# gk969/stm32-speech-recognition

Measured on NVIDIA H100. Metric: utterances/s, higher is better.
Workload: dtype int32 fixed-point (s16 FFT, u32 energies)

## Files before the change

stm32-speech-recognition_b200/csrc/sr_mfcc.cu:

```cuda
#include <stdio.h>
#include "sr_mfcc_core.cuh"

namespace srk {

constexpr int kPcmBufBytes = 19264;
__host__ __device__ constexpr int padF(int e) { return e + ((e >> 6) << 2); }
constexpr int kFftWords = 2 * (padF(1023) + 1);
static_assert(kFftWords >= kFftWordsTotal, "filter scratch must fit in the FFT buffer");

constexpr int kMfccWarps = 16;
constexpr int kNBuf = 3;

struct __align__(16) MfccSmem {
    unsigned char pcm[kNBuf][kPcmBufBytes];
    int2 tw[340 * 3];
    u32 log_thr[2220];
    u32 tri_even[512];
    u32 tri_odd[512];
    int4 dct[24 * 3];
    u32 fftbuf[kMfccWarps][kFftWords];
    s32 wq[kMfccWarps][160];
    u32 lg[kMfccWarps][32];
    u64 full[kNBuf];
    u64 empty[kNBuf];
    s32 meta[kNBuf][5];
    int turn;
};

static_assert(sizeof(MfccSmem) <= 232448, "mfcc_kernel_s16 exceeds the 227 KB shared-memory opt-in limit");

__device__ __forceinline__ void stage_utterance(MfccSmem &sm, int it, u32 b, const u16 *__restrict__ pcm,
                                                u32 U, const u32 *__restrict__ seg, u32 seg_stride,
                                                const atap_tag *__restrict__ atap, unsigned char *__restrict__ ftr,
                                                const u32 *__restrict__ row_map, size_t total_bytes, bool base_aligned,
                                                int lane) {
    const int s = it % kNBuf;
    const u32 st = seg[(size_t)b * seg_stride], en = seg[(size_t)b * seg_stride + 1];
    const u32 mid = atap[b].mid_val;
    const long long row = row_map ? (long long)row_map[b] : (long long)b;
    if (it >= kNBuf) mbar_wait(&sm.empty[s], ((it / kNBuf) - 1) & 1);
    const int F = mfcc_frames<SR_FRAME_LEN>(st, en, U);
    if (lane == 0) *reinterpret_cast<u16 *>(ftr + (size_t)b * kFtrBytes + 2) = (u16)F;
    if (F == 0) {
        if (lane == 0) {
            sm.meta[s][0] = 0; sm.meta[s][1] = 0; sm.meta[s][2] = (s32)mid; sm.meta[s][3] = (s32)b; sm.meta[s][4] = 0;
            mbar_arrive(&sm.full[s]);
        }
        return;
    }
    if (lane == 0) sm.meta[s][4] = (st == 0);
    long long first = row * U + st - 1;
    const long long last = row * U + st + 80ll * (F - 1) + 160;
    unsigned char *dst = sm.pcm[s];
    int off = 0;
    if (first < 0) {
        first = 0; off = 8;
        dst += 16;
    }
    const size_t lo = (size_t)first * 2, hi = (size_t)last * 2;
    if (base_aligned) {
        const size_t lo_al = lo & ~(size_t)15;
        size_t hi_al = (hi + 15) & ~(size_t)15;
        const size_t lim = total_bytes & ~(size_t)15;
        if (hi_al > lim) hi_al = lim;
        const u32 nbytes = (u32)(hi_al - lo_al);
        const int shift = (int)((lo - lo_al) >> 1);
        if (lane == 0) {
            sm.meta[s][0] = F; sm.meta[s][2] = (s32)mid; sm.meta[s][3] = (s32)b;
            sm.meta[s][1] = (off ? 7 : shift);
        }
        if (hi > hi_al) {
            const u16 *g = reinterpret_cast<const u16 *>(reinterpret_cast<const unsigned char *>(pcm) + hi_al);
            u16 *d = reinterpret_cast<u16 *>(dst + (hi_al - lo_al));
            const int n = (int)((hi - hi_al) >> 1);
            if (lane < n) d[lane] = g[lane];
        }
        __syncwarp();
        if (lane == 0) {
            mbar_arrive_expect_tx(&sm.full[s], nbytes);
            bulk_g2s(dst, reinterpret_cast<const unsigned char *>(pcm) + lo_al, nbytes, &sm.full[s]);
        }
    } else {
        const u16 *g = pcm + first;
        u16 *d = reinterpret_cast<u16 *>(dst);
        const int n = (int)(last - first);
        for (int i = lane; i < n; i += 32) d[i] = g[i];
        __syncwarp();
        if (lane == 0) {
            sm.meta[s][0] = F; sm.meta[s][2] = (s32)mid; sm.meta[s][1] = off ? 7 : 0; sm.meta[s][3] = (s32)b;
            mbar_arrive(&sm.full[s]);
        }
    }
}

__device__ __forceinline__ void stage_end(MfccSmem &sm, int it, int lane) {
    const int s = it % kNBuf;
    if (it >= kNBuf) mbar_wait(&sm.empty[s], ((it / kNBuf) - 1) & 1);
    if (lane == 0) { sm.meta[s][0] = -1; mbar_arrive(&sm.full[s]); }
}

__global__ void __maxnreg__(128) mfcc_kernel_s16(const u16 *__restrict__ pcm, u32 U, u32 B, const u32 *__restrict__ seg,
                                                 u32 seg_stride, const atap_tag *__restrict__ atap,
                                                 unsigned char *__restrict__ ftr, const DevTables *__restrict__ tab,
                                                 const u32 *__restrict__ row_map, u32 rows_total, const u32 *__restrict__ B_dev,
                                                 u32 *__restrict__ work ) {
    constexpr int kAhead = kNBuf - 2;
    if (B_dev) B = min(B, *B_dev);
    auto cta_done = [&]() {
        if (work && threadIdx.x == 0) {
            __threadfence();
            if (atomicAdd(&work[1], 1u) == gridDim.x - 1u) { work[0] = 0; work[1] = 0; }
        }
    };
    if (blockIdx.x >= B) { cta_done(); return; }
    extern __shared__ __align__(128) unsigned char smem_raw[];
    MfccSmem &sm = *reinterpret_cast<MfccSmem *>(smem_raw);
    const int warp = threadIdx.x >> 5, lane = threadIdx.x & 31;

    for (int i = threadIdx.x; i < 340 * 3; i += blockDim.x) sm.tw[i] = tab->tw[i];
    for (int i = threadIdx.x; i < 2220; i += blockDim.x) sm.log_thr[i] = tab->log_thr[i];
    for (int i = threadIdx.x; i < 24 * 12; i += blockDim.x)
        reinterpret_cast<s32 *>(sm.dct)[i] = (s32)tab->dct[(i / 24) * 24 + ((i / 12) & 1) * 12 + i % 12];
    for (int i = threadIdx.x; i < 512; i += blockDim.x) {
        sm.tri_even[flt_word(i >> 4, i & 15)] = tab->tri_even[i];
        sm.tri_odd[flt_word(i >> 4, i & 15)] = tab->tri_odd[i];
    }
    if (threadIdx.x == 0) {
        for (int s = 0; s < kNBuf; ++s) { mbar_init(&sm.full[s], 1); mbar_init(&sm.empty[s], kMfccWarps); }
        sm.turn = 0;
        mbar_fence_init();
    }
    __syncthreads();

    const size_t total_bytes = (size_t)(row_map ? rows_total : B) * U * 2;
    const bool base_aligned = (reinterpret_cast<uintptr_t>(pcm) & 15) == 0;

    auto claim_stage = [&](int it_s) {
        u32 b;
        if (work) {
            b = 0;
            if (lane == 0) {
                volatile int *turn = &sm.turn;
                while (*turn != it_s) { }
                b = atomicAdd(&work[0], 1u);
                __threadfence_block();
                if (b != 0xFFFFFFFFu) *turn = it_s + 1;
            }
            b = __shfl_sync(0xFFFFFFFFu, b, 0);
        }
        else b = blockIdx.x + (u32)it_s * gridDim.x;
        if (b < B) stage_utterance(sm, it_s, b, pcm, U, seg, seg_stride, atap, ftr, row_map, total_bytes, base_aligned, lane);
        else stage_end(sm, it_s, lane);
    };
    if (warp < kAhead) claim_stage(warp);

    u32 *fb = sm.fftbuf[warp];
    s32 *wq = sm.wq[warp];
    const int q1 = lane & 3;
    const int2 k1_2 = sm.tw[q1 * 3 + 1], k1_1 = sm.tw[q1 * 3 + 2];
    int2 k2t[4][3];
#pragma unroll
    for (int m1 = 0; m1 < 4; ++m1)
#pragma unroll
        for (int j = 0; j < 3; ++j) k2t[m1][j] = sm.tw[(4 + q1 + 4 * m1) * 3 + j];
    const u32 hm0 = tab->hamm[lane], hm1 = tab->hamm[lane + 32], hm2 = tab->hamm[lane + 64],
              hm3 = tab->hamm[lane + 96], hm4 = tab->hamm[lane + 128];
    const int fsw = (lane >> 1) & 3;
    int fe_lo = kFltZero, fe_hi = kFltZero, fx_lo = kFltX, fx_hi = kFltX;
    if (lane < 24) {
        fe_lo = tab->flt_e_lo[lane]; fe_hi = tab->flt_e_hi[lane];
        fx_lo = kFltX + (lane & 1) * 33 + tab->flt_x_lo[lane]; fx_hi = kFltX + (lane & 1) * 33 + tab->flt_x_hi[lane];
    }
    const int4 *dctk4 = sm.dct + 3 * (lane < 24 ? lane : 0);

    u32 gidx = 0;
    for (int it = 0;; ++it) {
        if (warp == it % kMfccWarps) claim_stage(it + kAhead);
        const int s = it % kNBuf;
        mbar_wait(&sm.full[s], (it / kNBuf) & 1);
        const int F = sm.meta[s][0];
        if (F < 0) break;
        const u32 b = (u32)sm.meta[s][3];
        const int off = sm.meta[s][1];
        const s32 mid = sm.meta[s][2];
        u16 *x = reinterpret_cast<u16 *>(sm.pcm[s]) + off;
        unsigned char *out_rows = ftr + (size_t)b * kFtrBytes + 4;
        const int f0 = (int)((warp - (int)(gidx % kMfccWarps) + kMfccWarps) % kMfccWarps);
        if (f0 == 0 && lane == 0 && sm.meta[s][4]) x[0] = (u16)mid;

        auto preemph = [&](const u16 *xf) {
            const u32 hm[5] = {hm0, hm1, hm2, hm3, hm4};
#pragma unroll
            for (int k = 0; k < 5; ++k) {
                const int i = lane + 32 * k;
                wq[i] = preemph_hamm(xf[i + 1], xf[i], (u32)mid, hm[k]) >> 2;
            }
        };
        for (int f = f0; f < F; f += kMfccWarps) {
            const u16 *xf = x + 80 * f;
            preemph(xf);
            __syncwarp();

#pragma unroll 1
            for (int pass = 0; pass < 2; ++pass) {
                const int G = (lane >> 2) + 8 * pass;
                const int r0 = (int)(__brev((u32)G) >> 28);
                u32 vr[4][4], vi[4][4];
#pragma unroll
                for (int m2 = 0; m2 < 4; ++m2) {
                    const int r = r0 + 16 * (((m2 & 1) << 1) | (m2 >> 1));
                    const u32 a = (u32)wq[r];
                    const u32 c = (u32)wq[r + 64];
                    u32 Cr, Ci, Br = 0, Bi = 0;
                    cxmul(Cr, Ci, c, 0u, (u32)k1_2.x, (u32)k1_2.y);
                    if ((m2 & 1) == 0) {
                        const u32 bb = (u32)wq[r + 128];
                        cxmul(Br, Bi, bb, 0u, (u32)k1_1.x, (u32)k1_1.y);
                    }
                    u32 o[8];
                    cxadda4<14>(a, 0u, Br, Bi, Cr, Ci, 0u, 0u, o[0], o[1], o[2], o[3], o[4], o[5], o[6], o[7]);
#pragma unroll
                    for (int m1 = 0; m1 < 4; ++m1) { vr[m2][m1] = o[2 * m1]; vi[m2][m1] = o[2 * m1 + 1]; }
                }
#pragma unroll
                for (int m1 = 0; m1 < 4; ++m1) {
                    const int q2 = q1 + 4 * m1;
                    const int2 k3 = k2t[m1][0], k2 = k2t[m1][1], k1 = k2t[m1][2];
                    u32 Dr, Di, Cr, Ci, Br, Bi;
                    cxmul(Dr, Di, vr[3][m1], vi[3][m1], (u32)k3.x, (u32)k3.y);
                    cxmul(Cr, Ci, vr[2][m1], vi[2][m1], (u32)k2.x, (u32)k2.y);
                    cxmul(Br, Bi, vr[1][m1], vi[1][m1], (u32)k1.x, (u32)k1.y);
                    u32 o[8];
                    cxadda4<14>(vr[0][m1], vi[0][m1], Br, Bi, Cr, Ci, Dr, Di, o[0], o[1], o[2], o[3], o[4], o[5], o[6], o[7]);
                    uint2 *dst = reinterpret_cast<uint2 *>(fb) + padF(64 * G + q2);
#pragma unroll
                    for (int m = 0; m < 4; ++m) dst[16 * m] = make_uint2(o[2 * m], o[2 * m + 1]);
                }
            }
            __syncwarp();

            u32 held[8];
#pragma unroll
            for (int pass = 0; pass < 2; ++pass) {
                const int q3 = lane + 32 * pass;
                u32 vr[4][4], vi[4][4];
                const int2 *k = &sm.tw[(20 + q3) * 3];
                const int2 k3 = k[0], k2 = k[1], k1 = k[2];
                const uint2 *pts = reinterpret_cast<const uint2 *>(fb) + padF(q3);
#pragma unroll
                for (int m4 = 0; m4 < 4; ++m4) {
                    u32 pr[4], pi[4];
#pragma unroll
                    for (int m3 = 0; m3 < 4; ++m3) {
                        const uint2 p = pts[padF(256 * m4 + 64 * m3)];
                        pr[m3] = p.x; pi[m3] = p.y;
                    }
                    u32 Dr, Di, Cr, Ci, Br, Bi;
                    cxmul(Dr, Di, pr[3], pi[3], (u32)k3.x, (u32)k3.y);
                    cxmul(Cr, Ci, pr[2], pi[2], (u32)k2.x, (u32)k2.y);
                    cxmul(Br, Bi, pr[1], pi[1], (u32)k1.x, (u32)k1.y);
                    u32 o[8];
                    cxadda4<14>(pr[0], pi[0], Br, Bi, Cr, Ci, Dr, Di, o[0], o[1], o[2], o[3], o[4], o[5], o[6], o[7]);
#pragma unroll
                    for (int m3 = 0; m3 < 4; ++m3) { vr[m4][m3] = o[2 * m3]; vi[m4][m3] = o[2 * m3 + 1]; }
                }
                __syncwarp();
                if (pass == 1) {
#pragma unroll
                    for (int m3 = 0; m3 < 4; ++m3) { fb[padF(lane + 64 * m3)] = held[2 * m3]; fb[padF(lane + 64 * m3 + 256)] = held[2 * m3 + 1]; }
                }
#pragma unroll
                for (int m3 = 0; m3 < 4; ++m3) {
                    const int q4 = q3 + 64 * m3;
                    const int2 *kk = &sm.tw[(84 + q4) * 3];
                    const int2 j3 = kk[0], j2 = kk[1], j1 = kk[2];
                    u32 Dr, Di, Cr, Ci, Br, Bi;
                    cxmul(Dr, Di, vr[3][m3], vi[3][m3], (u32)j3.x, (u32)j3.y);
                    cxmul(Cr, Ci, vr[2][m3], vi[2][m3], (u32)j2.x, (u32)j2.y);
                    cxmul(Br, Bi, vr[1][m3], vi[1][m3], (u32)j1.x, (u32)j1.y);
                    u32 o[8];
                    cxadda4<14>(vr[0][m3], vi[0][m3], Br, Bi, Cr, Ci, Dr, Di, o[0], o[1], o[2], o[3], o[4], o[5], o[6], o[7]);
                    const u32 m0 = mag10_small(o[0], o[1]);
                    const u32 m1 = mag10_small(o[2], o[3]);
                    if (pass == 0) { held[2 * m3] = m0 * m0; held[2 * m3 + 1] = m1 * m1; }
                    else { fb[padF(q4)] = m0 * m0; fb[padF(q4 + 256)] = m1 * m1; }
                }
            }
            __syncwarp();

            {
                u32 E[16];
                const uint4 *e4 = reinterpret_cast<const uint4 *>(fb + 16 * lane + 4 * (lane >> 2));
#pragma unroll
                for (int j = 0; j < 4; ++j) { const uint4 v = e4[j]; E[4 * j] = v.x; E[4 * j + 1] = v.y; E[4 * j + 2] = v.z; E[4 * j + 3] = v.w; }
                __syncwarp();
                const uint4 *we4 = reinterpret_cast<const uint4 *>(sm.tri_even + 16 * lane);
                const uint4 *wo4 = reinterpret_cast<const uint4 *>(sm.tri_odd + 16 * lane);
                uint4 *re4 = reinterpret_cast<uint4 *>(fb + 16 * lane);
                uint4 *ro4 = reinterpret_cast<uint4 *>(fb + kFltRowWords + 16 * lane);
                u32 te = 0, to = 0;
#pragma unroll
                for (int j = 0; j < 4; ++j) {
                    const uint4 we = we4[j ^ fsw], wo = wo4[j ^ fsw];
                    uint4 pe, po;
                    pe.x = te; te += (E[4 * j] * we.x) / 100u;      po.x = to; to += (E[4 * j] * wo.x) / 100u;
                    pe.y = te; te += (E[4 * j + 1] * we.y) / 100u;  po.y = to; to += (E[4 * j + 1] * wo.y) / 100u;
                    pe.z = te; te += (E[4 * j + 2] * we.z) / 100u;  po.z = to; to += (E[4 * j + 2] * wo.z) / 100u;
                    pe.w = te; te += (E[4 * j + 3] * we.w) / 100u;  po.w = to; to += (E[4 * j + 3] * wo.w) / 100u;
                    re4[j ^ fsw] = pe; ro4[j ^ fsw] = po;
                }
                fb[kFltX + lane] = te;
                fb[kFltX + 33 + lane] = to;
                fb[kFltZero] = 0u;
            }
            __syncwarp();
            {
                u32 acc = fb[fe_hi] - fb[fe_lo];
#pragma unroll
                for (int j = 0; j < 6; ++j) if (fx_lo + j < fx_hi) acc += fb[fx_lo + j];
                sm.lg[warp][lane] = (lane < 24) ? log100(acc, sm.log_thr) : 0u;
            }
            __syncwarp();
            {
                const int4 d0 = dctk4[0], d1 = dctk4[1], d2 = dctk4[2];
                const s32 dctk[12] = {d0.x, d0.y, d0.z, d0.w, d1.x, d1.y, d1.z, d1.w, d2.x, d2.y, d2.z, d2.w};
                dct_row(sm.lg[warp], dctk, out_rows + (size_t)f * kRowBytes, lane);
            }
            __syncwarp();
        }
        gidx += (u32)F;
        __syncwarp();
        if (lane == 0) mbar_arrive(&sm.empty[s]);
    }
    __syncthreads();
    cta_done();
}

__global__ void __launch_bounds__(128)
fft_generic_kernel(const u32 *__restrict__ in , const s16 *__restrict__ frames, u32 len,
                   u32 n, u32 *__restrict__ raw_out , u32 *__restrict__ mag ,
                   const DevTables *__restrict__ tab) {
    __shared__ u32 buf[4][1024];
    __shared__ u32 src[4][1024];
    const int warp = threadIdx.x >> 5, lane = threadIdx.x & 31;
    const u32 fr = blockIdx.x * 4 + warp;
    if (fr >= n) return;
    u32 *x = src[warp], *y = buf[warp];
    for (int i = lane; i < 1024; i += 32) {
        u32 v;
        if (in) v = in[(size_t)fr * 1024 + i];
        else v = (u32)i < len ? (u32)(u16)frames[(size_t)fr * len + i] : 0u;
        x[i] = v;
    }
    __syncwarp();
    fft_radix4<1024>(x, y, tab, lane);
    if (raw_out) for (int i = lane; i < 1024; i += 32) raw_out[(size_t)fr * 1024 + i] = y[i];
    if (mag) for (int i = lane; i < 512; i += 32) mag[(size_t)fr * 512 + i] = mag10(lo16s(y[i]), hi16s(y[i]));
}

cudaError_t launch_mfcc(const u16 *pcm, u32 U, u32 B, const u32 *seg, u32 seg_stride, const atap_tag *atap,
                        void *ftr, int num_sms, cudaStream_t st, const u32 *row_map, u32 rows_total, const u32 *B_dev, u32 *work) {
    if (B == 0) return cudaSuccess;
    const DevTables *tab = dev_tables();
    if (!tab) return cudaErrorInitializationError;
    const size_t smem = sizeof(MfccSmem);
    const int threads = kMfccWarps * 32;
    cudaError_t e = cudaFuncSetAttribute(mfcc_kernel_s16, cudaFuncAttributeMaxDynamicSharedMemorySize, (int)smem);
    if (e != cudaSuccess) return e;
    const u32 grid = B < (u32)num_sms ? B : (u32)num_sms;
    mfcc_kernel_s16<<<grid, threads, smem, st>>>(pcm, U, B, seg, seg_stride, atap, static_cast<unsigned char *>(ftr), tab,
                                                 row_map, rows_total, B_dev, work);
    e = cudaGetLastError();
    if (e != cudaSuccess) {
        cudaFuncAttributes fa;
        if (cudaFuncGetAttributes(&fa, mfcc_kernel_s16) == cudaSuccess)
            fprintf(stderr, "mfcc kernel launch failed (%s): regs %d, maxThreads %d, static smem %zu, dyn smem %zu (max %d), threads %d\n",
                    cudaGetErrorString(e), fa.numRegs, fa.maxThreadsPerBlock, fa.sharedSizeBytes, smem,
                    fa.maxDynamicSharedSizeBytes, threads);
    }
    return e;
}

cudaError_t launch_fft_generic(const u32 *in_packed, const s16 *frames, u32 len, u32 n, u32 *raw_out, u32 *mag,
                               cudaStream_t st) {
    if (n == 0) return cudaSuccess;
    const DevTables *tab = dev_tables();
    if (!tab) return cudaErrorInitializationError;
    fft_generic_kernel<<<(n + 3) / 4, 128, 0, st>>>(in_packed, frames, len, n, raw_out, mag, tab);
    return cudaGetLastError();
}

}
```

stm32-speech-recognition_b200/csrc/sr_mfcc_core.cuh:

```cuda
#pragma once
#include "sr_common.cuh"

namespace srk {

template <u32 kFrameLen>
__device__ __forceinline__ int mfcc_frames(u32 start, u32 end, u32 U) {
    if (start == SR_SEG_NULL || end == SR_SEG_NULL || end > U || start > end) return 0;
    u32 len = end - start;
    if (len < kFrameLen) return 0;
    u32 n = (len - kFrameLen) / SR_FRAME_MOV + 1u;
    return n > SR_VV_FRM_MAX ? 0 : (int)n;
}

__device__ __forceinline__ s32 preemph_hamm(u32 cur, u32 prv, u32 mid, u32 hamm) {
    const s32 c = (s32)(cur - mid), p = (s32)(prv - mid);
    const s32 t = (s32)((u32)c - (u32)((s32)((u32)p * 95u) / 100));
    return (s32)(s16)((s32)((u32)t * hamm) / 1000);
}

template <int N>
__device__ __forceinline__ void fft_radix4(const u32 *x, u32 *y, const DevTables *tab, int lane) {
    static_assert(N == 256 || N == 1024, "the twiddle table serves N = 256 and 1024");
    constexpr int kQ = N / 4, kRevShift = N == 256 ? 26 : 24;
    for (int idx = lane; idx < kQ; idx += 32) {
        const int j = (int)(__brev((u32)idx) >> kRevShift);
        const u32 A = x[j], C = x[j + kQ], Bv = x[j + 2 * kQ], D = x[j + 3 * kQ];
        u32 o[8];
        cxadda4<0>(lo16s(A), hi16s(A), lo16s(Bv), hi16s(Bv), lo16s(C), hi16s(C), lo16s(D), hi16s(D),
                   o[0], o[1], o[2], o[3], o[4], o[5], o[6], o[7]);
#pragma unroll
        for (int m = 0; m < 4; ++m) y[4 * idx + m] = pack16(o[2 * m], o[2 * m + 1]);
    }
    __syncwarp();
    int toff = 0;
    for (int s = 4; s <= kQ; s <<= 2) {
        for (int t = lane; t < kQ; t += 32) {
            const int q = t % s, base = (t / s) * 4 * s;
            const int2 k3 = tab->tw[(toff + q) * 3], k2 = tab->tw[(toff + q) * 3 + 1], k1 = tab->tw[(toff + q) * 3 + 2];
            const u32 p0 = y[base + q], p1 = y[base + q + s], p2 = y[base + q + 2 * s], p3 = y[base + q + 3 * s];
            u32 Dr, Di, Cr, Ci, Br, Bi, o[8];
            cxmul(Dr, Di, lo16s(p3), hi16s(p3), (u32)k3.x, (u32)k3.y);
            cxmul(Cr, Ci, lo16s(p2), hi16s(p2), (u32)k2.x, (u32)k2.y);
            cxmul(Br, Bi, lo16s(p1), hi16s(p1), (u32)k1.x, (u32)k1.y);
            cxadda4<14>(lo16s(p0), hi16s(p0), Br, Bi, Cr, Ci, Dr, Di, o[0], o[1], o[2], o[3], o[4], o[5], o[6], o[7]);
#pragma unroll
            for (int m = 0; m < 4; ++m) y[base + q + m * s] = pack16(o[2 * m], o[2 * m + 1]);
        }
        __syncwarp();
        toff += s;
    }
}

__device__ __forceinline__ u32 log100(u32 v, const u32 *thr) {
    if (v == 0) return 0;
    int L = (int)(__log2f(__uint2float_rn(v)) * 69.31471805599453f);
    L = max(0, min(L, 2218));
    while (v < thr[L]) --L;
    while (L < 2218 && v >= thr[L + 1]) ++L;
    return (u32)L;
}

__device__ __forceinline__ void dct_row(const u32 *lg, const s32 (&w)[12], unsigned char *row, int lane) {
    const u32 *lgp = lg + (lane & 1) * 12;
    s32 acc = 0;
#pragma unroll
    for (int i = 0; i < 12; ++i) acc += ((s32)lgp[i] * w[i]) / 100;
    acc += __shfl_xor_sync(0xFFFFFFFFu, acc, 1);
    if (lane < 24 && (lane & 1) == 0) *reinterpret_cast<s16 *>(row + (lane >> 1) * 2) = (s16)acc;
}

}
```

Before: 11.39 million.

## Batch log and DCT tail across frames with mulhi-based division

Filterbank energies are buffered per warp for four frames, then log100 and the DCT run as one batch so all 32 lanes do useful work instead of 24. The per-term divide by 100 in the DCT becomes a __mulhi with pre-scaled weights plus a count of negative terms as a rounding correction. log100 gets branchless single-step corrections, and the window buffer shrinks to s16 with explicit sign-extending loads. The single-step correction assumes the float estimate is off by at most one, and the mulhi trick must reproduce truncating division exactly.

Result: faster. 11.56 million (median of 6 runs) (+1.5%).

```diff
diff --git a/stm32-speech-recognition_b200/csrc/sr_mfcc.cu b/stm32-speech-recognition_b200/csrc/sr_mfcc.cu
--- a/stm32-speech-recognition_b200/csrc/sr_mfcc.cu
+++ b/stm32-speech-recognition_b200/csrc/sr_mfcc.cu
@@ -5,11 +5,17 @@
 
 constexpr int kPcmBufBytes = 19264;
 __host__ __device__ constexpr int padF(int e) { return e + ((e >> 6) << 2); }
+__device__ __forceinline__ u32 lds_s16(const s16 *p) {
+    s32 v;
+    asm volatile("ld.shared.s16 %0, [%1];" : "=r"(v) : "r"(smem_u32(p)) : "memory");
+    return (u32)v;
+}
 constexpr int kFftWords = 2 * (padF(1023) + 1);
 static_assert(kFftWords >= kFftWordsTotal, "filter scratch must fit in the FFT buffer");
 
 constexpr int kMfccWarps = 16;
 constexpr int kNBuf = 3;
+constexpr int kFrameBatch = 4;
 
 struct __align__(16) MfccSmem {
     unsigned char pcm[kNBuf][kPcmBufBytes];
@@ -18,9 +24,11 @@
     u32 tri_even[512];
     u32 tri_odd[512];
     int4 dct[24 * 3];
+    s32 dct_neg[24];
     u32 fftbuf[kMfccWarps][kFftWords];
-    s32 wq[kMfccWarps][160];
-    u32 lg[kMfccWarps][32];
+    s16 wq[kMfccWarps][160];
+    u32 tail[kMfccWarps][kFrameBatch * 24];
+    unsigned char *rows[kMfccWarps][kFrameBatch];
     u64 full[kNBuf];
     u64 empty[kNBuf];
     s32 meta[kNBuf][5];
@@ -119,8 +127,12 @@
 
     for (int i = threadIdx.x; i < 340 * 3; i += blockDim.x) sm.tw[i] = tab->tw[i];
     for (int i = threadIdx.x; i < 2220; i += blockDim.x) sm.log_thr[i] = tab->log_thr[i];
-    for (int i = threadIdx.x; i < 24 * 12; i += blockDim.x)
-        reinterpret_cast<s32 *>(sm.dct)[i] = (s32)tab->dct[(i / 24) * 24 + ((i / 12) & 1) * 12 + i % 12];
+    for (int i = threadIdx.x; i < 24 * 12; i += blockDim.x) reinterpret_cast<s32 *>(sm.dct)[i] = (s32)tab->dct[i] * kDctM;
+    if (threadIdx.x < 24) {
+        s32 n = 0;
+        for (int i = 0; i < 12; ++i) n += tab->dct[12 * threadIdx.x + i] < 0;
+        sm.dct_neg[threadIdx.x] = n;
+    }
     for (int i = threadIdx.x; i < 512; i += blockDim.x) {
         sm.tri_even[flt_word(i >> 4, i & 15)] = tab->tri_even[i];
         sm.tri_odd[flt_word(i >> 4, i & 15)] = tab->tri_odd[i];
@@ -155,7 +167,8 @@
     if (warp < kAhead) claim_stage(warp);
 
     u32 *fb = sm.fftbuf[warp];
-    s32 *wq = sm.wq[warp];
+    s16 *wq = sm.wq[warp];
+    u32 *tl = sm.tail[warp];
     const int q1 = lane & 3;
     const int2 k1_2 = sm.tw[q1 * 3 + 1], k1_1 = sm.tw[q1 * 3 + 2];
     int2 k2t[4][3];
@@ -171,7 +184,29 @@
         fe_lo = tab->flt_e_lo[lane]; fe_hi = tab->flt_e_hi[lane];
         fx_lo = kFltX + (lane & 1) * 33 + tab->flt_x_lo[lane]; fx_hi = kFltX + (lane & 1) * 33 + tab->flt_x_hi[lane];
     }
-    const int4 *dctk4 = sm.dct + 3 * (lane < 24 ? lane : 0);
+
+    auto tail_batch = [&](int n) {
+        __syncwarp();
+#pragma unroll
+        for (int k = 0; k < 3; ++k) tl[32 * k + lane] = dct_lg(log100(tl[32 * k + lane], sm.log_thr));
+        __syncwarp();
+#pragma unroll 1
+        for (int k = 0; k < 3; ++k) {
+            const int c = 16 * k + (lane >> 1), fr = c / 12, role = 2 * (c - 12 * fr) + (lane & 1);
+            const int4 *w4 = sm.dct + 3 * role;
+            const int4 *l4 = reinterpret_cast<const int4 *>(tl + 24 * fr + 12 * (lane & 1));
+            s32 acc = sm.dct_neg[role];
+#pragma unroll
+            for (int j = 0; j < 3; ++j) {
+                const int4 w = w4[j], l = l4[j];
+                acc += __mulhi(l.x, w.x); acc += __mulhi(l.y, w.y); acc += __mulhi(l.z, w.z); acc += __mulhi(l.w, w.w);
+            }
+            acc += __shfl_xor_sync(0xFFFFFFFFu, acc, 1);
+            if ((lane & 1) == 0 && fr < n) *reinterpret_cast<s16 *>(sm.rows[warp][fr] + (c - 12 * fr) * 2) = (s16)acc;
+        }
+        __syncwarp();
+    };
+    int nb = 0;
 
     u32 gidx = 0;
     for (int it = 0;; ++it) {
@@ -209,12 +244,12 @@
 #pragma unroll
                 for (int m2 = 0; m2 < 4; ++m2) {
                     const int r = r0 + 16 * (((m2 & 1) << 1) | (m2 >> 1));
-                    const u32 a = (u32)wq[r];
-                    const u32 c = (u32)wq[r + 64];
+                    const u32 a = lds_s16(wq + r);
+                    const u32 c = lds_s16(wq + r + 64);
                     u32 Cr, Ci, Br = 0, Bi = 0;
                     cxmul(Cr, Ci, c, 0u, (u32)k1_2.x, (u32)k1_2.y);
                     if ((m2 & 1) == 0) {
-                        const u32 bb = (u32)wq[r + 128];
+                        const u32 bb = lds_s16(wq + r + 128);
                         cxmul(Br, Bi, bb, 0u, (u32)k1_1.x, (u32)k1_1.y);
                     }
                     u32 o[8];
@@ -318,20 +353,17 @@
                 u32 acc = fb[fe_hi] - fb[fe_lo];
 #pragma unroll
                 for (int j = 0; j < 6; ++j) if (fx_lo + j < fx_hi) acc += fb[fx_lo + j];
-                sm.lg[warp][lane] = (lane < 24) ? log100(acc, sm.log_thr) : 0u;
-            }
+                if (lane < 24) tl[24 * nb + lane] = acc;
+                if (lane == 0) sm.rows[warp][nb] = out_rows + (size_t)f * kRowBytes;
+            }
+            if (++nb == kFrameBatch) { tail_batch(nb); nb = 0; }
             __syncwarp();
-            {
-                const int4 d0 = dctk4[0], d1 = dctk4[1], d2 = dctk4[2];
-                const s32 dctk[12] = {d0.x, d0.y, d0.z, d0.w, d1.x, d1.y, d1.z, d1.w, d2.x, d2.y, d2.z, d2.w};
-                dct_row(sm.lg[warp], dctk, out_rows + (size_t)f * kRowBytes, lane);
-            }
-            __syncwarp();
         }
         gidx += (u32)F;
         __syncwarp();
         if (lane == 0) mbar_arrive(&sm.empty[s]);
     }
+    if (nb) tail_batch(nb);
     __syncthreads();
     cta_done();
 }
diff --git a/stm32-speech-recognition_b200/csrc/sr_mfcc_core.cuh b/stm32-speech-recognition_b200/csrc/sr_mfcc_core.cuh
--- a/stm32-speech-recognition_b200/csrc/sr_mfcc_core.cuh
+++ b/stm32-speech-recognition_b200/csrc/sr_mfcc_core.cuh
@@ -52,13 +52,15 @@
 }
 
 __device__ __forceinline__ u32 log100(u32 v, const u32 *thr) {
-    if (v == 0) return 0;
     int L = (int)(__log2f(__uint2float_rn(v)) * 69.31471805599453f);
     L = max(0, min(L, 2218));
-    while (v < thr[L]) --L;
-    while (L < 2218 && v >= thr[L + 1]) ++L;
-    return (u32)L;
+    L -= (int)(v < thr[L]);
+    L += (int)(L < 2218 && v >= thr[L + 1]);
+    return v == 0 ? 0u : (u32)L;
 }
+
+constexpr s32 kDctM = 10737419;
+__device__ __forceinline__ u32 dct_lg(u32 lg) { return lg ? 4u * lg : 1u; }
 
 __device__ __forceinline__ void dct_row(const u32 *lg, const s32 (&w)[12], unsigned char *row, int lane) {
     const u32 *lgp = lg + (lane & 1) * 12;
```
